# zwyang6/ExCEL

Measured on AMD Instinct MI355X. Metric: images/sec (CAM+PAR refine, 448x448), higher is better.
Workload: dtype bf16x3 (fp32 as bf16 hi+lo, fp32 accumulate)

## Files before the change

### excel_amd/csrc/abi.hip

```cpp
#include "../../include/excel_hip.h"
#include "common.h"
#include "excel_internal.h"

#include <stdarg.h>
#include <map>
#include <vector>

static thread_local char g_err[512] = "";

void excel_set_error(const char* fmt, ...) {
    va_list ap;
    va_start(ap, fmt);
    vsnprintf(g_err, sizeof(g_err), fmt, ap);
    va_end(ap);
}

extern "C" const char* excel_last_error(void) { return g_err; }
extern "C" int excel_abi_version(void) { return 5; }
#ifndef EXCEL_BUILD_ID
#define EXCEL_BUILD_ID "unstamped"
#endif
extern "C" const char* excel_build_id(void) { return EXCEL_BUILD_ID; }

bool g_excel_prof_on = false;
// ... 532 lines not shown

extern "C" size_t excel_cam_workspace_bytes(int B, int N, int T) {
    return align_up((size_t)B * N * ((T + 3) / 4 * 4) * sizeof(float), 256);
}

extern "C" int excel_clip_feature_surgery(const float* image_features, const float* text, int B, int N, int C, int T, int F,
                                          float temperature, float* out_full, float* out_slice, void* workspace, void* stream) {
    EXCEL_CHECK_ARG(image_features && text && workspace && (out_full || out_slice), "clip_feature_surgery: null argument");
    EXCEL_CHECK_ARG((C % 4) == 0, "clip_feature_surgery: C must be a multiple of 4");
    const int ldT = (T + 3) / 4 * 4;
    float* S = (float*)workspace;
    GemmArgs ga = gemm_args(image_features, text, S, nullptr, nullptr, B * N, T, C, C, C, ldT, 0, GEMM_ACT_NONE);
    TRY(excel_launch_gemm(ga, true, 1, ST(stream)));
    return excel_launch_cam_epilogue(S, out_full, out_slice, B, N, T, ldT, F, temperature, ST(stream));
}

struct PtcWs { float *sim, *part, *colsq; unsigned short* ts; size_t total; };
static PtcWs ptc_ws_layout(int B, int N, int C, int T, char* base) {
    PtcWs w;
    size_t off = 0;
    auto take = [&](size_t bytes) { char* p = base + off; off += align_up(bytes, 256); return p; };
    w.sim = (float*)take(excel_patch_text_cam_ws_floats(B, N, C, T, 0) * sizeof(float));
    w.ts = (unsigned short*)take((size_t)T * C * sizeof(float));
    w.part = (float*)take(excel_patch_text_cam_ws_floats(B, N, C, T, 1) * sizeof(float));
    w.colsq = (float*)take(excel_patch_text_cam_ws_floats(B, N, C, T, 2) * sizeof(float));
    w.total = off;
    return w;
}
extern "C" size_t excel_patch_text_cam_workspace_bytes(int B, int N, int C, int T) { return ptc_ws_layout(B, N, C, T, nullptr).total; }

extern "C" int excel_patch_text_cam(const float* x_raw, const float* text, int B, int N, int C, int T, int F, float temperature, int mode,
                                    float* out_full, float* out_slice, float* image_features, void* workspace, void* stream) {
    EXCEL_CHECK_ARG(x_raw && text && workspace && (out_full || out_slice), "patch_text_cam: null argument");
    EXCEL_CHECK_ARG(mode == 0 || mode == 1 || mode == 2, "patch_text_cam: mode must be 0 (exact fp32), 1 (bf16x3) or 2 (f16x3)");
    EXCEL_CHECK_ARG(B > 0 && N > 0 && C > 0 && T > 0, "patch_text_cam: bad shape");
    const int ldT = (T + 3) / 4 * 4;
    const PtcWs w = ptc_ws_layout(B, N, C, T, (char*)workspace);
    if (mode == 2)
        return excel_f16::excel_launch_patch_text_cam(x_raw, text, w.ts, w.sim, w.part, w.colsq, out_full, out_slice, image_features, B, N, C, T, F,
                                                      ldT, temperature, 1, ST(stream));
    return excel_launch_patch_text_cam(x_raw, text, mode == 1 ? w.ts : nullptr, w.sim, w.part, w.colsq, out_full, out_slice, image_features, B, N, C,
                                       T, F, ldT, temperature, mode, ST(stream));
}

extern "C" int excel_attn_layer_mean(const float* attn, int Lw, int B, int N, int first_layer, int n_layers, float* w_aff, void* stream) {
    EXCEL_CHECK_ARG(attn && w_aff && first_layer >= 0 && n_layers >= 1 && first_layer + n_layers <= Lw, "attn_layer_mean: bad layer range");
    const long long n = (long long)B * (N - 1) * (N - 1);
    hipLaunchKernelGGL(attn_layer_mean_kernel, dim3((unsigned)cdivl(n, 256)), dim3(256), 0, ST(stream), attn, B, N, first_layer, n_layers, w_aff);
    EXCEL_CHECK_LAUNCH("attn_layer_mean");
    return EXCEL_OK;
}

extern "C" size_t excel_trans_mat_workspace_bytes(int B, int P) {
    return 2 * align_up((size_t)B * P * P * sizeof(float), 256) + align_up((size_t)B * P * sizeof(float), 256);
}

extern "C" int excel_compute_trans_mat(const float* w_aff, int B, int P, float* trans_out, void* workspace, void* stream) {
    EXCEL_CHECK_ARG(w_aff && trans_out && workspace, "compute_trans_mat: null argument");
    EXCEL_CHECK_ARG((P % 4) == 0, "compute_trans_mat: P must be a multiple of 4 (P=%d)", P);
    char* base = (char*)workspace;
    const size_t mat = align_up((size_t)B * P * P * sizeof(float), 256);
    float* T = (float*)base;
    float* Tsym = (float*)(base + mat);
    float* cs = (float*)(base + 2 * mat);
    TRY(excel_launch_trans_mat_sym(w_aff, T, Tsym, cs, B, P, ST(stream)));
    GemmArgs ga = gemm_args(Tsym, Tsym, trans_out, nullptr, nullptr, P, P, P, P, P, P, 0, GEMM_ACT_NONE);
    ga.sA = ga.sB = ga.sC = (long long)P * P;
    return excel_launch_gemm(ga, true, B, ST(stream));
}

extern "C" int excel_cls_compact(const float* onehot, int B, int F, int Smax, int32_t* cls_idx, int32_t* ncls, int32_t* nchan,
                                 void* stream) {
    EXCEL_CHECK_ARG(onehot && cls_idx && ncls && Smax >= 1, "cls_compact: bad argument");
    return excel_launch_cls_compact(onehot, B, F, Smax, cls_idx, ncls, nchan, ST(stream));
}

extern "C" int excel_scoremap_box_mask(const float* attr, const int32_t* cls_idx, const int32_t* ncls, int B, int g, int F, int Smax,
                                       double caa_thre, float* v_out, uint8_t* mask_out, void* stream) {
    EXCEL_CHECK_ARG(attr && cls_idx && ncls && v_out, "scoremap_box_mask: null argument");
    return excel_launch_bbox_mask(attr, cls_idx, ncls, B, g, F, Smax, caa_thre, v_out, mask_out, ST(stream));
}

extern "C" size_t excel_refine_workspace_bytes(int B, int P, int Smax) {
    return 2 * align_up((size_t)B * P * P * sizeof(float), 256) + align_up((size_t)B * P * sizeof(float), 256) +
           2 * align_up((size_t)B * Smax * P * sizeof(float), 256);
}

extern "C" int excel_refine_cams_with_aff(const float* attr, const float* w_aff, const int32_t* cls_idx, const int32_t* ncls, int B,
                                          int g, int F, int Smax, double caa_thre, float* refined, void* workspace, void* stream) {
    EXCEL_CHECK_ARG(attr && w_aff && cls_idx && ncls && refined && workspace, "refine_cams_with_aff: null argument");
    const int P = g * g;
    char* base = (char*)workspace;
    const size_t mat = align_up((size_t)B * P * P * sizeof(float), 256);
    const size_t vec = align_up((size_t)B * Smax * P * sizeof(float), 256);
    float* T = (float*)base;
    float* Tsym = (float*)(base + mat);
    float* cs = (float*)(base + 2 * mat);
    float* v = (float*)(base + 2 * mat + align_up((size_t)B * P * sizeof(float), 256));
    float* u = (float*)((char*)v + vec);
    hipStream_t st = ST(stream);
    TRY(excel_launch_trans_mat_sym(w_aff, T, Tsym, cs, B, P, st));
    TRY(excel_launch_bbox_mask(attr, cls_idx, ncls, B, g, F, Smax, caa_thre, v, nullptr, st));
    TRY(excel_launch_matvec(Tsym, v, ncls, u, B, P, Smax, st));
    TRY(excel_launch_matvec(Tsym, u, ncls, refined, B, P, Smax, st));
    return EXCEL_OK;
}

extern "C" int excel_cam_upsample_bkg(const float* refined, const int32_t* ncls, int B, int g, int Smax, int H, int W, float* cams,
                                      void* workspace, int flags, void* stream) {
    EXCEL_CHECK_ARG(refined && ncls && cams && workspace, "cam_upsample_bkg: null argument");
    return excel_launch_cam_upsample_bkg(refined, ncls, (float*)workspace, cams, B, g, Smax, H, W, (flags & EXCEL_CAMS_ZERO_UNUSED) ? 1 : 0, ST(stream));
}

extern "C" int excel_ragged_plan(const int32_t* hw, int B, excel_ragged_info* info, int32_t* table) {
    EXCEL_CHECK_ARG(hw && info && B >= 1, "ragged_plan: bad argument");
    long long pix = 0, lab = 0, tiles = 0, max_plane = 0;
    for (int b = 0; b < B; ++b) {
        const long long H = hw[2 * b], W = hw[2 * b + 1];
        EXCEL_CHECK_ARG(H >= 1 && W >= 1, "ragged_plan: image %d has size %lld x %lld", b, H, W);
        const long long Wp = (W + 3) / 4 * 4, plane = H * Wp, nt = ((W + 63) / 64) * ((H + 15) / 16);
        if (table) {
            int32_t* rec = table + EXCEL_RAG_REC * b;
            rec[0] = (int32_t)H; rec[1] = (int32_t)W; rec[2] = (int32_t)pix; rec[3] = (int32_t)tiles; rec[4] = (int32_t)lab; rec[5] = rec[6] = rec[7] = 0;
            for (long long t = 0; t < nt; ++t) table[EXCEL_RAG_REC * (B + 1) + tiles + t] = b;
        }
        pix += plane; lab += H * W; tiles += nt;
        if (plane > max_plane) max_plane = plane;
        EXCEL_CHECK_ARG(pix < (1LL << 31) && 3 * lab < (1LL << 31) && tiles < (1LL << 31), "ragged_plan: batch too large for 32-bit offsets");
    }
    if (table) {
        int32_t* rec = table + EXCEL_RAG_REC * B;
        rec[0] = rec[1] = 0; rec[2] = (int32_t)pix; rec[3] = (int32_t)tiles; rec[4] = (int32_t)lab; rec[5] = rec[6] = rec[7] = 0;
    }
    info->B = B; info->total_tiles = (int32_t)tiles; info->total_pix = pix; info->total_label_pix = lab; info->max_plane_pix = max_plane;
    info->table_ints = EXCEL_RAG_REC * (long long)(B + 1) + tiles;
    return EXCEL_OK;
}

static TileGeo ragged_geo(const int32_t* table, int B) {
    TileGeo g;
    g.tab = table; g.B = B; g.H = g.W = 0;
    return g;
}
static TileGeo uniform_geo(int B, int H, int W) {
    TileGeo g;
    g.tab = nullptr; g.B = B; g.H = H; g.W = W;
    return g;
}

extern "C" int excel_normalize_resize_u8_ragged(const uint8_t* hwc, const int32_t* table, int B, int S, const double* mean3, const double* std3,
                                                float* out, void* stream) {
    EXCEL_CHECK_ARG(hwc && table && out && mean3 && std3 && B > 0 && S > 0, "normalize_resize_u8_ragged: bad argument");
    return excel_launch_normalize_resize_u8_ragged(hwc, out, ragged_geo(table, B), S, mean3, std3, ST(stream));
}

extern "C" int excel_normalize_resize_u8_ragged_mirror(const uint8_t* hwc, const int32_t* table, int B, int S, const double* mean3,
                                                       const double* std3, float* out, void* stream) {
    EXCEL_CHECK_ARG(hwc && table && out && mean3 && std3 && B > 0 && S > 0, "normalize_resize_u8_ragged_mirror: bad argument");
    return excel_launch_normalize_resize_u8_ragged_mirror(hwc, out, ragged_geo(table, B), S, mean3, std3, ST(stream));
}

extern "C" int excel_cam_upsample_bkg_ragged(const float* refined, const int32_t* ncls, const int32_t* table, const excel_ragged_info* info, int g,
                                             int Smax, float* cams, void* workspace, int flags, void* stream) {
    EXCEL_CHECK_ARG(refined && ncls && table && info && cams && workspace, "cam_upsample_bkg_ragged: null argument");
    EXCEL_CHECK_ARG((((uintptr_t)cams) & 15) == 0, "cam_upsample_bkg_ragged: cams must be 16-byte aligned");
    return excel_launch_cam_upsample_bkg_ragged(refined, ncls, (float*)workspace, cams, g, Smax, ragged_geo(table, info->B), info->total_tiles,
                                                (flags & EXCEL_CAMS_ZERO_UNUSED) ? 1 : 0, ST(stream));
}

int excel_aug_plan(const int32_t* hw, const excel_aug_params* prm, int B, int S, excel_train_aug_info* info, int32_t* table);
int excel_launch_train_augment(const unsigned char* hwc, const unsigned char* labels, const int* table, const excel_train_aug_info& info,
                               const double* mean, const double* stdv, float* img, unsigned char* label, int* img_box, void* workspace,
                               hipStream_t st);
int excel_launch_train_augment_image(const unsigned char* hwc, const int* table, const excel_train_aug_info& info, const double* mean,
                                     const double* stdv, float* img, int* img_box, void* workspace, hipStream_t st);
extern "C" int excel_train_aug_plan(const int32_t* hw, const excel_aug_params* params, int B, int S, excel_train_aug_info* info, int32_t* table) {
    return excel_aug_plan(hw, params, B, S, info, table);
}

extern "C" size_t excel_train_augment_workspace_bytes(const excel_train_aug_info* info) {
    return info ? (size_t)info->workspace_bytes : 0;
}

extern "C" int excel_train_augment(const uint8_t* hwc, const uint8_t* labels, const int32_t* table, const excel_train_aug_info* info,
                                   const double* mean3, const double* std3, float* img, uint8_t* label, int32_t* img_box, void* workspace,
                                   void* stream) {
    EXCEL_CHECK_ARG(hwc && labels && table && info && mean3 && std3 && img && label && img_box && workspace, "train_augment: null argument");
    EXCEL_CHECK_ARG(info->B >= 1 && info->S >= 1 && info->max_h >= 1 && info->max_w2 >= 1 && info->workspace_bytes > 0,
// ... 144 lines not shown
```

### excel_amd/csrc/aff.hip

```cpp
#include "common.h"
#include "excel_internal.h"

__global__ __launch_bounds__(256) void colsum_kernel(const float* __restrict__ T, float* __restrict__ cs, int P) {
    __shared__ float part[4][64];
    const int b = blockIdx.y, cl = threadIdx.x & 63, g = threadIdx.x >> 6;
    const int c = blockIdx.x * 64 + cl;
    const float* Tb = T + (long long)b * P * P;
    float a8[8] = {0.f, 0.f, 0.f, 0.f, 0.f, 0.f, 0.f, 0.f};
    if (c < P) {
        int i = g;
        for (; i + 28 < P; i += 32) {
#pragma unroll
            for (int u = 0; u < 8; ++u) a8[u] += Tb[(long long)(i + 4 * u) * P + c];
        }
        for (int u = 0; i < P; i += 4, ++u) a8[u] += Tb[(long long)i * P + c];
    }
    const float s = ((a8[0] + a8[1]) + (a8[2] + a8[3])) + ((a8[4] + a8[5]) + (a8[6] + a8[7]));
    part[g][cl] = s;
    __syncthreads();
    if (g == 0 && c < P) cs[(long long)b * P + c] = (part[0][cl] + part[1][cl]) + (part[2][cl] + part[3][cl]);
}

#define SK_MAXP 2048
__global__ __launch_bounds__(256) void sinkhorn_row_kernel(const float* __restrict__ in, const float* __restrict__ cs,
// ... 67 lines not shown
    const int cls = cls_idx[(long long)b * Smax + s];
    const int P = g * g;
    if (tid == 0) { s_max = 0; s_nroots = 0; }
    __syncthreads();
    int u8v[BB_MAXP / 256];
#pragma unroll
    for (int k = 0; k < BB_MAXP / 256; ++k) {
        const int p = tid + 256 * k;
        u8v[k] = 0;
        if (p < P) {
            const float x = attr[((long long)b * P + p) * F + cls];
            gv[p] = x;
            u8v[k] = (int)(x * 255.f) & 255;
            atomicMax(&s_max, u8v[k]);
        }
    }
    __syncthreads();
    const int thr = (int)(thre * (double)s_max);
#pragma unroll
    for (int k = 0; k < BB_MAXP / 256; ++k) {
        const int p = tid + 256 * k;
        if (p < P) {
            lab[p] = (u8v[k] > thr) ? p : -1;
            bx0[p] = g; bx1[p] = -1; by0[p] = g; by1[p] = -1;
        }
    }
    __syncthreads();
    for (int iter = 0; iter < 2 * BB_MAXP; ++iter) {
        if (tid == 0) s_changed = 0;
        __syncthreads();
#pragma unroll
        for (int k = 0; k < BB_MAXP / 256; ++k) {
            const int p = tid + 256 * k;
            if (p < P && lab[p] >= 0) {
                const int y = p / g, x = p % g;
                int best = lab[p];
                for (int dy = -1; dy <= 1; ++dy)
                    for (int dx = -1; dx <= 1; ++dx) {
                        const int yy = y + dy, xx = x + dx;
                        if (yy >= 0 && yy < g && xx >= 0 && xx < g) {
                            const int l2 = lab[yy * g + xx];
                            if (l2 >= 0 && l2 < best) best = l2;
                        }
                    }
                const int jump = lab[best];
                if (jump >= 0 && jump < best) best = jump;
                if (best < lab[p]) { atomicMin(&lab[p], best); s_changed = 1; }
            }
        }
        __syncthreads();
        if (!s_changed) break;
        __syncthreads();
    }
#pragma unroll
    for (int k = 0; k < BB_MAXP / 256; ++k) {
        const int p = tid + 256 * k;
        if (p < P && lab[p] >= 0) {
            const int root = lab[p], y = p / g, x = p % g;
            atomicMin(&bx0[root], x); atomicMax(&bx1[root], x);
            atomicMin(&by0[root], y); atomicMax(&by1[root], y);
            if (root == p) roots[atomicAdd(&s_nroots, 1)] = p;
        }
    }
    __syncthreads();
    const int nroots = s_nroots;
#pragma unroll
    for (int k = 0; k < BB_MAXP / 256; ++k) {
        const int p = tid + 256 * k;
        if (p < P) {
            const int y = p / g, x = p % g;
            bool in = false;
            for (int i = 0; i < nroots; ++i) {
                const int rt = roots[i];
                const int x1 = min(bx1[rt] + 1, g - 1), y1 = min(by1[rt] + 1, g - 1);
                in = in || (x >= bx0[rt] && x < x1 && y >= by0[rt] && y < y1);
            }
            v_out[((long long)b * Smax + s) * P + p] = in ? gv[p] : 0.f;
            if (mask_out) mask_out[((long long)b * Smax + s) * P + p] = in ? 1 : 0;
        }
    }
}

#define MV_S 8
__global__ __launch_bounds__(256) void matvec_kernel(const float* __restrict__ T, const float* __restrict__ v,
                                                     const int* __restrict__ ncls, float* __restrict__ u, int P, int Smax,
                                                     int s0) {
    extern __shared__ float vs[];
    const int b = blockIdx.y;
    const int ns = min(min(ncls[b], Smax) - s0, MV_S);
    if (ns <= 0) return;
    for (int i = threadIdx.x; i < ns * P; i += 256) vs[i] = v[((long long)b * Smax + s0) * P + i];
    __syncthreads();
    const int lane = threadIdx.x & 63, wave = threadIdx.x >> 6;
    for (int rr = 0; rr < 4; ++rr) {
        const int i = blockIdx.x * 16 + wave * 4 + rr;
        if (i >= P) break;
        const float* row = T + ((long long)b * P + i) * P;
        float acc[MV_S];
#pragma unroll
        for (int s = 0; s < MV_S; ++s) acc[s] = 0.f;
        for (int j = lane; j < P; j += 64) {
            const float t = row[j];
#pragma unroll
            for (int s = 0; s < MV_S; ++s)
                if (s < ns) acc[s] += t * vs[s * P + j];
        }
#pragma unroll
        for (int s = 0; s < MV_S; ++s) {
            if (s < ns) {
                const float r = wave_sum(acc[s]);
                if (lane == 0) u[((long long)b * Smax + s0 + s) * P + i] = r;
            }
        }
    }
}

__global__ __launch_bounds__(256) void cam_minmax_norm_kernel(const float* __restrict__ r, const int* __restrict__ ncls,
                                                              float* __restrict__ rn, int P, int Smax) {
    __shared__ float smn[4], smx[4];
    const int s = blockIdx.x, b = blockIdx.y;
    if (s >= min(ncls[b], Smax)) return;
    const float* src = r + ((long long)b * Smax + s) * P;
    float mn = INFINITY, mx = -INFINITY;
    for (int p = threadIdx.x; p < P; p += 256) { const float v = src[p]; mn = fminf(mn, v); mx = fmaxf(mx, v); }
    mn = wave_min(mn); mx = wave_max(mx);
    if ((threadIdx.x & 63) == 0) { smn[threadIdx.x >> 6] = mn; smx[threadIdx.x >> 6] = mx; }
    __syncthreads();
    mn = fminf(fminf(smn[0], smn[1]), fminf(smn[2], smn[3]));
    mx = fmaxf(fmaxf(smx[0], smx[1]), fmaxf(smx[2], smx[3]));
    const float den = 1e-7f + (mx - mn);
    float* dst = rn + ((long long)b * Smax + s) * P;
    for (int p = threadIdx.x; p < P; p += 256) dst[p] = (src[p] - mn) / den;
}

struct CvTap { int s0, s1; float f; };
__device__ __forceinline__ CvTap cv_linear_tap(int d, int g, int D) {
    const double fd = ((double)d + 0.5) * ((double)g / (double)D) - 0.5;
    CvTap t;
    t.s0 = (int)floor(fd);
    t.f = (float)(fd - t.s0);
    if (t.s0 < 0) { t.f = 0.f; t.s0 = 0; }
    if (t.s0 >= g - 1) { t.f = 0.f; t.s0 = g - 1; }
    t.s1 = min(t.s0 + 1, g - 1);
    return t;
}
__device__ __forceinline__ void cam_upsample_px(const float* __restrict__ rn_b, float* __restrict__ out, long long HW, int g, int ns, int Smax,
                                                const CvTap& tx, const CvTap& ty, int zero_unused) {
    float mx = -INFINITY;
    for (int s = 0; s < ns; ++s) {
        const float* m = rn_b + (long long)s * g * g;
        const float top = fmaf(m[ty.s0 * g + tx.s1], tx.f, __fmul_rn(m[ty.s0 * g + tx.s0], 1.f - tx.f));
        const float bot = fmaf(m[ty.s1 * g + tx.s1], tx.f, __fmul_rn(m[ty.s1 * g + tx.s0], 1.f - tx.f));
        const float v = fmaf(bot, ty.f, __fmul_rn(top, 1.f - ty.f));
        out[(long long)(s + 1) * HW] = v;
        mx = fmaxf(mx, v);
    }
    out[0] = 1.f - mx;
    if (zero_unused)
        for (int s = ns; s < Smax; ++s) out[(long long)(s + 1) * HW] = 0.f;
}

__global__ __launch_bounds__(256) void cam_upsample_bkg_kernel(const float* __restrict__ rn, const int* __restrict__ ncls,
                                                               float* __restrict__ cams, int g, int Smax, int H, int W, int zero_unused) {
    const int b = blockIdx.z;
    const int x = blockIdx.x * 64 + (threadIdx.x & 63);
    const int y = blockIdx.y * 4 + (threadIdx.x >> 6);
    if (x >= W || y >= H) return;
    const int ns = min(ncls[b], Smax);
    const long long HW = (long long)H * W;
    cam_upsample_px(rn + (long long)b * Smax * g * g, cams + (long long)b * (Smax + 1) * HW + (long long)y * W + x, HW, g, ns, Smax,
                    cv_linear_tap(x, g, W), cv_linear_tap(y, g, H), zero_unused);
}

__global__ __launch_bounds__(256) void cam_upsample_bkg_ragged_kernel(const float* __restrict__ rn, const int* __restrict__ ncls,
                                                                      float* __restrict__ cams, int g, int Smax, TileGeo geo, int zero_unused) {
    const Tile t = tile_of<true>(geo);
    const int x = t.x0 + (threadIdx.x & 63);
    if (x >= t.W) return;
    const int ns = min(ncls[t.b], Smax);
    const CvTap tx = cv_linear_tap(x, g, t.W);
    const float* rn_b = rn + (long long)t.b * Smax * g * g;
    float* cb = cams + (long long)(Smax + 1) * t.base + x;
#pragma unroll 1
    for (int r = 0; r < 4; ++r) {
        const int y = t.y0 + (threadIdx.x >> 6) + 4 * r;
        if (y < t.H) cam_upsample_px(rn_b, cb + (long long)y * t.Wp, t.HW, g, ns, Smax, tx, cv_linear_tap(y, g, t.H), zero_unused);
    }
}

int excel_launch_trans_mat_sym(const float* W, float* T, float* Tsym, float* cs, int B, int P, hipStream_t st) {
    ProfScope prof__(PROF_SINKHORN, st);
    EXCEL_CHECK_ARG(P <= SK_MAXP, "compute_trans_mat: P=%d exceeds %d", P, SK_MAXP);
    const float* src = W;
    for (int round = 0; round < 3; ++round) {
        hipLaunchKernelGGL(colsum_kernel, dim3(cdiv(P, 64), B), dim3(256), 0, st, src, cs, P);
        hipLaunchKernelGGL(sinkhorn_row_kernel, dim3(cdiv(P, 4), B), dim3(256), 0, st, src, cs, T, P);
        src = T;
    }
    hipLaunchKernelGGL(symmetrize_kernel, dim3(cdiv(P, 32), cdiv(P, 32), B), dim3(256), 0, st, T, Tsym, P);
    EXCEL_CHECK_LAUNCH("trans_mat_sym");
    return EXCEL_OK;
}

int excel_launch_cls_compact(const float* onehot, int B, int F, int Smax, int* cls_idx, int* ncls, int* nchan, hipStream_t st) {
    ProfScope prof__(PROF_OTHER, st);
    hipLaunchKernelGGL(cls_compact_kernel, dim3(cdiv(B, 64)), dim3(64), 0, st, onehot, B, F, Smax, cls_idx, ncls, nchan);
    EXCEL_CHECK_LAUNCH("cls_compact");
    return EXCEL_OK;
}

int excel_launch_bbox_mask(const float* attr, const int* cls_idx, const int* ncls, int B, int g, int F, int Smax, double thre,
                           float* v_out, unsigned char* mask_out, hipStream_t st) {
    ProfScope prof__(PROF_BBOX, st);
    EXCEL_CHECK_ARG(g * g <= BB_MAXP, "scoremap2bbox: grid %dx%d exceeds %d cells", g, g, BB_MAXP);
    hipLaunchKernelGGL(bbox_mask_kernel, dim3(Smax, B), dim3(256), 0, st, attr, cls_idx, ncls, g, F, Smax, thre, v_out, mask_out);
    EXCEL_CHECK_LAUNCH("bbox_mask");
    return EXCEL_OK;
}

int excel_launch_matvec(const float* T, const float* v, const int* ncls, float* u, int B, int P, int Smax, hipStream_t st) {
    ProfScope prof__(PROF_MATVEC, st);
    for (int s0 = 0; s0 < Smax; s0 += MV_S) {
        hipLaunchKernelGGL(matvec_kernel, dim3(cdiv(P, 16), B), dim3(256), MV_S * P * sizeof(float), st, T, v, ncls, u, P, Smax, s0);
    }
    EXCEL_CHECK_LAUNCH("matvec");
    return EXCEL_OK;
}

int excel_launch_cam_upsample_bkg(const float* r, const int* ncls, float* rn, float* cams, int B, int g, int Smax, int H, int W,
                                  int zero_unused, hipStream_t st) {
    ProfScope prof__(PROF_UPSAMPLE, st);
    hipLaunchKernelGGL(cam_minmax_norm_kernel, dim3(Smax, B), dim3(256), 0, st, r, ncls, rn, g * g, Smax);
    hipLaunchKernelGGL(cam_upsample_bkg_kernel, dim3(cdiv(W, 64), cdiv(H, 4), B), dim3(256), 0, st, rn, ncls, cams, g, Smax, H, W, zero_unused);
    EXCEL_CHECK_LAUNCH("cam_upsample_bkg");
    return EXCEL_OK;
}

int excel_launch_cam_upsample_bkg_ragged(const float* r, const int* ncls, float* rn, float* cams, int g, int Smax, const TileGeo& geo,
                                         int total_tiles, int zero_unused, hipStream_t st) {
    ProfScope prof__(PROF_UPSAMPLE, st);
    hipLaunchKernelGGL(cam_minmax_norm_kernel, dim3(Smax, geo.B), dim3(256), 0, st, r, ncls, rn, g * g, Smax);
    hipLaunchKernelGGL(cam_upsample_bkg_ragged_kernel, dim3(total_tiles), dim3(256), 0, st, rn, ncls, cams, g, Smax, geo, zero_unused);
    EXCEL_CHECK_LAUNCH("cam_upsample_bkg_ragged");
    return EXCEL_OK;
}
```

### excel_amd/csrc/excel_internal.h

```cpp
#pragma once
#include <hip/hip_runtime.h>

enum { GEMM_ACT_NONE = 0, GEMM_ACT_QUICKGELU = 1, GEMM_ACT_RELU = 2 };
enum { GEMM_OUT_PLAIN = 0, GEMM_OUT_QKV_HEADMAJOR = 1, GEMM_OUT_SPLIT_BF16 = 2 };

struct GemmArgs {
    const float* A;
    const float* B;
    float* C;
    const float* bias;
    const float* res;
    int M, N, K;
    int Kld;
    int lda, ldb, ldc, ldr;
    long long sA, sB, sC, sR, sBias;
    int zdiv;
    long long sA2, sB2, sC2;
    int act;
    int out_mode;
    int tokN, heads, hd;
    float alpha;
};


// ... 2 lines not shown
    const unsigned short* B;
    float* C;
    unsigned short* Cs;
    const float* bias;
    const float* res;
    int M, N, K;
    int lda, ldb, ldc, ldr;
    int act, out_mode;
    int tokN, heads, hd;
    unsigned short* qkv_split;
    int dbg;
    int batch;
    long long sA, sB, sC, sCs;
    int mix_tall, mix_short;
    int mix_first;
    int w_lo_zero;
    const unsigned short* Bh;
    int ldbh;
};

struct GemmShape {
    int M, N, K, lda, ldb, ldc, ldr, hd, out_mode, has_residual, batch;
    int f16;
    int w_lo_zero;
    int half_ok;
};
enum { GEMM_8WAVE = 0, GEMM_8WAVE_MIXED = 1, GEMM_W4 = 2, GEMM_W4_MIX = 3 };
struct GemmPlan {
    int kernel;
    int tile;
    int nt_m;
    int x2;
    int tall, shrt, second;
    int grid_x, grid_y, block;
};
constexpr int GEMM_W4_BN = 256;
GemmPlan gemm_plan(const GemmShape& s, int n_cu);
enum { ATTN_STRIP = 0, ATTN_TWOPASS_SPLIT = 1, ATTN_TWOPASS_F32 = 2 };
constexpr int ATTN_STRIP_MAX_TILES = 40;
struct AttnPlan {
    int path;
    int ntiles;
    int ntw, nw, nw_full;
    int rp_ntypes;
    int rp_grid[3];
    int grid[3], block;
    int split_c;
};
AttnPlan attn_plan(int B, int H, int N, int gemm_mode, int surgery, int want_w);
enum { CAM_NARROW = 0, CAM_WIDE = 1 };
constexpr int PTC_MAXCT = 4;
constexpr int PTC_WIDE_T = 512;
constexpr int PTC_NW = 4;
constexpr int PTC_HB = 64;
constexpr int PTC_TLDS_ROWS = 48;
constexpr int PTC_TLDS_C = 512;
struct CamPlan {
    int kernel;
    int split;
    int ct;
    int tlds;
    int G;
    int prep_grid[3];
    int sim_grid[2], block;
    int finish_grid[2];
    int finish_pitch;
};
CamPlan cam_plan(int B, int N, int C, int T, int gemm_mode);
inline bool gemm_half_ok(bool aligned, int N, int K, int ldbh) {
    return aligned && ldbh >= K && (ldbh & 7) == 0 && (long long)N * ldbh * 2 < 0x7fffffffLL;
}

int excel_launch_gemm(const GemmArgs& p, bool b_kmajor, int batch, hipStream_t stream);
int excel_launch_attn_rowpass_f32(const float* qkvh, float* out, float* stats, int B, int H, int N, int hd, float scale,
                                  const AttnPlan& plan, hipStream_t st, int flash_nq);
int excel_launch_attn_accum_f32(const float* qkvh, const float* stats, float* a_sum, float* w_aff, float* attn_out, int B, int H,
                                int N, int NP, int hd, float scale, int surgery, float w_scale, float aff_scale, int aff_init,
                                const AttnPlan& plan, hipStream_t st, const float* ex_attn);

int excel_launch_trans_mat_sym(const float* W, float* T, float* Tsym, float* cs, int B, int P, hipStream_t st);
int excel_launch_cls_compact(const float* onehot, int B, int F, int Smax, int* cls_idx, int* ncls, int* nchan, hipStream_t st);
int excel_launch_bbox_mask(const float* attr, const int* cls_idx, const int* ncls, int B, int g, int F, int Smax, double thre,
                           float* v_out, unsigned char* mask_out, hipStream_t st);
int excel_launch_matvec(const float* T, const float* v, const int* ncls, float* u, int B, int P, int Smax, hipStream_t st);
int excel_launch_cam_upsample_bkg(const float* r, const int* ncls, float* rn, float* cams, int B, int g, int Smax, int H, int W,
                                  int zero_unused, hipStream_t st);
struct TileGeo;
int excel_launch_par_affinity(const float* img, float* aff, const TileGeo& geo, int total_tiles, const int* dil, int ndil, float w1, float w2,
                              hipStream_t st, int compact = 0);
int excel_par_guide_supported(const void* guide, const void* stats, const void* in, const void* out, int Cmax, long long max_plane, int Wp,
                              const int* dil, int ndil);
int excel_launch_par_iterate_guide(const float* guide, const float* stats, const float* in, float* out, const int* nchan, int Cmax,
                                   const TileGeo& geo, int total_tiles, const int* dil, int ndil, float w1, float w2, hipStream_t st);
int excel_launch_par_iterate(const float* aff, const float* in, float* out, const int* nchan, int B, int Cmax, int H, int W,
                             const int* dil, int ndil, hipStream_t st);
int excel_launch_bilinear_ac_ragged(const float* in, float* out, int h, int w, const TileGeo& geo, int total_tiles, hipStream_t st);
int excel_launch_argmax_label_ragged(const float* cams, const int* nchan, const int* cls_idx, int Smax, int Cmax, const TileGeo& geo,
                                     int total_tiles, unsigned char* lab8, hipStream_t st);
int excel_launch_cam_upsample_bkg_ragged(const float* r, const int* ncls, float* rn, float* cams, int g, int Smax, const TileGeo& geo,
                                         int total_tiles, int zero_unused, hipStream_t st);
int excel_launch_normalize_resize_u8_ragged(const unsigned char* hwc, float* out, const TileGeo& geo, int S, const double* mean, const double* stdv,
                                            hipStream_t st);
int excel_launch_normalize_resize_u8_ragged_mirror(const unsigned char* hwc, float* out, const TileGeo& geo, int S, const double* mean,
                                                   const double* stdv, hipStream_t st);
int excel_launch_bilinear_ac(const float* in, float* out, int planes, int h, int w, int H, int W, hipStream_t st);
int excel_launch_argmax_label(const float* cams, const int* nchan, const int* cls_idx, int B, int Smax, int Cmax, long long HW,
                              unsigned char* lab8, long long* lab64, hipStream_t st);
int excel_launch_confusion(const unsigned char* gt, const unsigned char* pred, long long n, int nc, unsigned long long* hist,
                           hipStream_t st);
int excel_launch_attr_aggregate(const float* text, const float* bank, int F, int T, int C, int K, int drop, float* out,
                                hipStream_t st);
int excel_launch_bilinear_resize(const float* in, float* out, long long planes, int h, int w, int H, int W, int align_corners,
                                 hipStream_t st);
int excel_launch_flip_max_normalize(const float* attr, float* out, int B, int g, int F, hipStream_t st);
int excel_launch_lam_scale_accumulate(const float* maps, float* acc, int B, int g, int F, int H, int W, int init, hipStream_t st);
int excel_launch_plane_minmax_normalize(float* lam, long long planes, long long HW, hipStream_t st);
int excel_launch_seg_scale_accumulate(const float* segs, float* acc, int B, int nc, int h, int w, int H, int W, int flip_mean, int init,
                                      float scale, hipStream_t st);
int excel_launch_denormalize(const float* img, unsigned char* out8, float* outf, int B, long long HW, const float* mean, const float* stdv,
                             hipStream_t st);
int excel_launch_normalize_u8(const unsigned char* hwc, float* out, int B, long long HW, const double* mean, const double* stdv, hipStream_t st);
int excel_launch_lam_to_label(const float* cam, const float* cls, const int* box, int B, int F, int H, int W, float bkg, float high, float low,
                              int ignore_mid, int ignore, float* valid, unsigned char* lab, hipStream_t st);
size_t excel_train_losses_ws_bytes(int B, int nc, int H, int W);
int excel_launch_train_losses(const float* seg, const float* attn_pred, const unsigned char* pseudo, const unsigned char* aff_labels, int B, int nc,
                              int g_h, int g_w, int H, int W, int radius, int ignore, float w_seg, float w_diver, float* losses, float* d_seg,
                              float* d_attn_pred, void* ws, hipStream_t st);
size_t excel_feature_affinity_ws_bytes(int B, int C, int P);
int excel_launch_feature_affinity(const float* feats, int B, int C, int P, float beta, float gamma, int mode, float* out, void* ws,
                                  hipStream_t st);
size_t excel_feature_affinity_grouped_ws_bytes(int B, int C, int P, int group);
int excel_launch_feature_affinity_grouped(const float* feats, int B, int C, int P, int group, int member_stride, float beta, float gamma,
                                          int mode, float* out, void* ws, hipStream_t st);
size_t excel_attn_select_ws_bytes(int B, int n_layers);
int excel_launch_attn_select_mean(const float* attn, int Lw, int B, int N, int first_layer, int n_layers, const float* seg_attn,
                                  float* out, void* ws, hipStream_t st);

namespace excel_bf16 {
#include "excel_split_api.inc"
}
namespace excel_f16 {
#include "excel_split_api.inc"
}
#ifdef EXCEL_SPLIT_F16
#define EXCEL_SPLIT_NS excel_f16
#else
#define EXCEL_SPLIT_NS excel_bf16
#endif
using namespace excel_bf16;

struct BilinearTap { int y0, y1, x0, x1; float ly, lx; };
__device__ __forceinline__ BilinearTap bilinear_tap(int x, int y, int h, int w, int H, int W, int align_corners) {
    float fy, fx;
    if (align_corners) {
        fy = ((H > 1) ? (float)(h - 1) / (float)(H - 1) : 0.f) * (float)y;
        fx = ((W > 1) ? (float)(w - 1) / (float)(W - 1) : 0.f) * (float)x;
    } else {
        fy = fmaxf(__fsub_rn(__fmul_rn((float)h / (float)H, (float)y + 0.5f), 0.5f), 0.f);
        fx = fmaxf(__fsub_rn(__fmul_rn((float)w / (float)W, (float)x + 0.5f), 0.5f), 0.f);
    }
    BilinearTap t;
    t.y0 = min((int)fy, h - 1); t.x0 = min((int)fx, w - 1);
    t.y1 = min(t.y0 + 1, h - 1); t.x1 = min(t.x0 + 1, w - 1);
    t.ly = fy - (float)t.y0; t.lx = fx - (float)t.x0;
    return t;
}
__device__ __forceinline__ float bilinear_blend(const BilinearTap& t, float p00, float p01, float p10, float p11) {
// ... 5 lines not shown
```

Before: 1493.

## Fuse Sinkhorn normalization and symmetrization into on-the-fly random-walk passes

Replaces the materialized transition matrix T and symmetric Tsym (two B×P×P buffers built by trans_mat_sym) with streaming passes over the raw affinity W. The passes compute row and column normalizers on the fly and apply the symmetric average as (row-half + column-half)/2, using per-block partial sums and a finish kernel. This removes the P×P intermediate writes and reads and the separate matvec kernel. In exchange it rereads W several times, adds more launches and partial-sum buffers, and reorders the floating-point arithmetic.

```diff
diff --git a/excel_amd/csrc/abi.hip b/excel_amd/csrc/abi.hip
--- a/excel_amd/csrc/abi.hip
+++ b/excel_amd/csrc/abi.hip
@@ -638,28 +638,14 @@
 }
 
 extern "C" size_t excel_refine_workspace_bytes(int B, int P, int Smax) {
-    return 2 * align_up((size_t)B * P * P * sizeof(float), 256) + align_up((size_t)B * P * sizeof(float), 256) +
-           2 * align_up((size_t)B * Smax * P * sizeof(float), 256);
+    return excel_refine_walk_workspace_bytes(B, P, Smax);
 }
 
 extern "C" int excel_refine_cams_with_aff(const float* attr, const float* w_aff, const int32_t* cls_idx, const int32_t* ncls, int B,
                                           int g, int F, int Smax, double caa_thre, float* refined, void* workspace, void* stream) {
     EXCEL_CHECK_ARG(attr && w_aff && cls_idx && ncls && refined && workspace, "refine_cams_with_aff: null argument");
-    const int P = g * g;
-    char* base = (char*)workspace;
-    const size_t mat = align_up((size_t)B * P * P * sizeof(float), 256);
-    const size_t vec = align_up((size_t)B * Smax * P * sizeof(float), 256);
-    float* T = (float*)base;
-    float* Tsym = (float*)(base + mat);
-    float* cs = (float*)(base + 2 * mat);
-    float* v = (float*)(base + 2 * mat + align_up((size_t)B * P * sizeof(float), 256));
-    float* u = (float*)((char*)v + vec);
-    hipStream_t st = ST(stream);
-    TRY(excel_launch_trans_mat_sym(w_aff, T, Tsym, cs, B, P, st));
-    TRY(excel_launch_bbox_mask(attr, cls_idx, ncls, B, g, F, Smax, caa_thre, v, nullptr, st));
-    TRY(excel_launch_matvec(Tsym, v, ncls, u, B, P, Smax, st));
-    TRY(excel_launch_matvec(Tsym, u, ncls, refined, B, P, Smax, st));
-    return EXCEL_OK;
+    EXCEL_CHECK_ARG(B >= 1 && g >= 1 && Smax >= 1, "refine_cams_with_aff: bad shape");
+    return excel_launch_refine_walk(attr, w_aff, cls_idx, ncls, B, g, F, Smax, caa_thre, refined, workspace, ST(stream));
 }
 
 extern "C" int excel_cam_upsample_bkg(const float* refined, const int32_t* ncls, int B, int g, int Smax, int H, int W, float* cams,
diff --git a/excel_amd/csrc/aff.hip b/excel_amd/csrc/aff.hip
--- a/excel_amd/csrc/aff.hip
+++ b/excel_amd/csrc/aff.hip
@@ -173,37 +173,180 @@
 }
 
 #define MV_S 8
-__global__ __launch_bounds__(256) void matvec_kernel(const float* __restrict__ T, const float* __restrict__ v,
-                                                     const int* __restrict__ ncls, float* __restrict__ u, int P, int Smax,
-                                                     int s0) {
-    extern __shared__ float vs[];
-    const int b = blockIdx.y;
-    const int ns = min(min(ncls[b], Smax) - s0, MV_S);
-    if (ns <= 0) return;
-    for (int i = threadIdx.x; i < ns * P; i += 256) vs[i] = v[((long long)b * Smax + s0) * P + i];
-    __syncthreads();
-    const int lane = threadIdx.x & 63, wave = threadIdx.x >> 6;
-    for (int rr = 0; rr < 4; ++rr) {
-        const int i = blockIdx.x * 16 + wave * 4 + rr;
-        if (i >= P) break;
-        const float* row = T + ((long long)b * P + i) * P;
-        float acc[MV_S];
-#pragma unroll
-        for (int s = 0; s < MV_S; ++s) acc[s] = 0.f;
-        for (int j = lane; j < P; j += 64) {
-            const float t = row[j];
-#pragma unroll
-            for (int s = 0; s < MV_S; ++s)
-                if (s < ns) acc[s] += t * vs[s * P + j];
-        }
-#pragma unroll
-        for (int s = 0; s < MV_S; ++s) {
-            if (s < ns) {
-                const float r = wave_sum(acc[s]);
-                if (lane == 0) u[((long long)b * Smax + s0 + s) * P + i] = r;
-            }
-        }
-    }
+#define RW_WAVE_ROWS 8
+__device__ __forceinline__ float walk_colsum(const float* __restrict__ p, int n, long long stride) {
+    float a = 0.f;
+    int k = 0;
+    for (; k + 4 <= n; k += 4) {
+        const float t0 = p[k * stride], t1 = p[(k + 1) * stride], t2 = p[(k + 2) * stride], t3 = p[(k + 3) * stride];
+        a = (((a + t0) + t1) + t2) + t3;
+    }
+    for (; k < n; ++k) a += p[k * stride];
+    return a;
+}
+
+template <int RB, int NK>
+__device__ __forceinline__ void walk_load_rows(float (&t)[RB][NK], const float* __restrict__ W, int b, int P, int i0, int lane) {
+#pragma unroll
+    for (int q = 0; q < RB; ++q) {
+        const int i = i0 + q;
+        const float* row = W + ((long long)b * P + min(i, P - 1)) * P;
+#pragma unroll
+        for (int k = 0; k < NK; ++k) {
+            const int j = lane + 64 * k;
+            t[q][k] = (64 * k < P && j < P && i < P) ? row[j] : 0.f;
+        }
+    }
+}
+
+template <bool RINV, bool HASX, int NK, int THREADS>
+__global__ __launch_bounds__(THREADS, (HASX || NK > 13) ? 2 : 4) void walk_pass_kernel(
+    const float* __restrict__ W, const float* __restrict__ cin, int nin, float* r, const float* __restrict__ x, const int* __restrict__ ncls,
+    float* __restrict__ rowhalf, float* __restrict__ part, int P, int Smax, int s0) {
+    extern __shared__ float lds[];
+    constexpr int NS = HASX ? 4 : 1, SLOTS = HASX ? MV_S : 1;
+    constexpr int RB = HASX ? 2 : 4;
+    constexpr bool PREFETCH = HASX;
+    constexpr int ROWS = THREADS / 64 * RW_WAVE_ROWS;
+    const int b = blockIdx.y, blk = blockIdx.x, nblk = gridDim.x, tid = threadIdx.x;
+    int ns = 1;
+    if (HASX) {
+        ns = min(min(ncls[b], Smax) - s0, MV_S);
+        if (ns <= 0) return;
+    }
+    float* cs = lds;
+    float* cxs = lds + P;
+    float* red = lds + (1 + ns) * P;
+    float* rrow = red + NS * P;
+    float* xrow = rrow + ROWS;
+    const float* xb = HASX ? x + ((long long)b * Smax + s0) * P : nullptr;
+    for (int j = tid; j < P; j += THREADS) {
+        const float c = 1.f / walk_colsum(cin + (long long)b * nin * P + j, nin, P);
+        cs[j] = c;
+        if (HASX)
+            for (int s = 0; s < ns; ++s) cxs[s * P + j] = c * xb[s * P + j];
+    }
+    if (HASX) {
+        for (int e = tid; e < (1 + ns) * ROWS; e += THREADS) {
+            const int s = e / ROWS - 1, i = blk * ROWS + e % ROWS;
+            if (s >= 0) rrow[e] = (i < P) ? xb[s * P + i] : 0.f;
+            else if (!RINV) rrow[e] = (i < P) ? r[(long long)b * P + i] : 0.f;
+        }
+    }
+    __syncthreads();
+    const int lane = tid & 63, wave = tid >> 6;
+    const int l0 = wave * RW_WAVE_ROWS, i0 = blk * ROWS + l0;
+    for (int sb = 0; sb < ns; sb += NS) {
+        float cacc[NS][NK];
+#pragma unroll
+        for (int s = 0; s < NS; ++s)
+#pragma unroll
+            for (int k = 0; k < NK; ++k) cacc[s][k] = 0.f;
+        float t[RB][NK], tn[RB][NK];
+        if (PREFETCH) walk_load_rows<RB, NK>(t, W, b, P, i0, lane);
+        for (int rr = 0; rr < RW_WAVE_ROWS; rr += RB) {
+            if (PREFETCH) {
+                if (rr + RB < RW_WAVE_ROWS) walk_load_rows<RB, NK>(tn, W, b, P, i0 + rr + RB, lane);
+            } else {
+                walk_load_rows<RB, NK>(t, W, b, P, i0 + rr, lane);
+            }
+            float d[RB], dx[RB][NS];
+#pragma unroll
+            for (int q = 0; q < RB; ++q) {
+                d[q] = 0.f;
+#pragma unroll
+                for (int s = 0; s < NS; ++s) dx[q][s] = 0.f;
+            }
+            if (RINV) {
+#pragma unroll
+                for (int k = 0; k < NK; ++k)
+                    if (64 * k < P) {
+                        const float c = cs[min(lane + 64 * k, P - 1)];
+#pragma unroll
+                        for (int q = 0; q < RB; ++q) d[q] = fmaf(t[q][k], c, d[q]);
+                    }
+            }
+            if (HASX) {
+#pragma unroll
+                for (int s = 0; s < NS; ++s)
+                    if (sb + s < ns) {
+#pragma unroll
+                        for (int k = 0; k < NK; ++k)
+                            if (64 * k < P) {
+                                const float cx = cxs[(sb + s) * P + min(lane + 64 * k, P - 1)];
+#pragma unroll
+                                for (int q = 0; q < RB; ++q) dx[q][s] = fmaf(t[q][k], cx, dx[q][s]);
+                            }
+                    }
+            }
+#pragma unroll
+            for (int q = 0; q < RB; ++q) {
+                if (RINV) d[q] = wave_sum(d[q]);
+                if (HASX) {
+#pragma unroll
+                    for (int s = 0; s < NS; ++s) dx[q][s] = wave_sum(dx[q][s]);
+                }
+            }
+#pragma unroll
+            for (int q = 0; q < RB; ++q) {
+                const int li = l0 + rr + q, i = i0 + rr + q;
+                const bool live = i < P;
+                float ri = 0.f;
+                if (RINV) {
+                    if (live) ri = 1.f / d[q];
+                    if (live && lane == 0 && sb == 0) r[(long long)b * P + i] = ri;
+                } else {
+                    ri = rrow[li];
+                }
+#pragma unroll
+                for (int s = 0; s < NS; ++s) {
+                    if (sb + s < ns && live) {
+                        float w = ri;
+                        if (HASX) {
+                            if (lane == 0) rowhalf[((long long)b * Smax + s0 + sb + s) * P + i] = ri * dx[q][s];
+                            w = ri * xrow[(sb + s) * ROWS + li];
+                        }
+#pragma unroll
+                        for (int k = 0; k < NK; ++k) cacc[s][k] = fmaf(t[q][k], w, cacc[s][k]);
+                    }
+                }
+            }
+            if (PREFETCH) {
+#pragma unroll
+                for (int q = 0; q < RB; ++q)
+#pragma unroll
+                    for (int k = 0; k < NK; ++k) t[q][k] = tn[q][k];
+            }
+        }
+        const int nv = min(ns - sb, NS);
+        for (int w = 0; w < THREADS / 64; ++w) {
+            if (wave == w) {
+#pragma unroll
+                for (int s = 0; s < NS; ++s)
+                    if (s < nv) {
+#pragma unroll
+                        for (int k = 0; k < NK; ++k) {
+                            const int j = lane + 64 * k;
+                            if (j < P) red[s * P + j] = (w == 0) ? cacc[s][k] : red[s * P + j] + cacc[s][k];
+                        }
+                    }
+            }
+            __syncthreads();
+        }
+        float* dst = part + (((long long)b * nblk + blk) * SLOTS + sb) * P;
+        for (int e = tid; e < nv * P; e += THREADS) dst[e] = red[e];
+        __syncthreads();
+    }
+}
+
+__global__ __launch_bounds__(256) void walk_apply_fin_kernel(const float* __restrict__ part, const float* __restrict__ cin, int nin,
+                                                             const int* __restrict__ ncls, float* __restrict__ y, int P, int nblk, int Smax,
+                                                             int s0) {
+    const int b = blockIdx.z, s = blockIdx.y, j = blockIdx.x * 256 + threadIdx.x;
+    if (j >= P || s >= min(min(ncls[b], Smax) - s0, MV_S)) return;
+    const float a = walk_colsum(part + ((long long)b * nblk * MV_S + s) * P + j, nblk, (long long)MV_S * P);
+    float* dst = y + ((long long)b * Smax + s0 + s) * P + j;
+    *dst = (*dst + (1.f / walk_colsum(cin + (long long)b * nin * P + j, nin, P)) * a) / 2.f;
 }
 
 __global__ __launch_bounds__(256) void cam_minmax_norm_kernel(const float* __restrict__ r, const int* __restrict__ ncls,
@@ -309,12 +452,62 @@
     return EXCEL_OK;
 }
 
-int excel_launch_matvec(const float* T, const float* v, const int* ncls, float* u, int B, int P, int Smax, hipStream_t st) {
+template <bool RINV, bool HASX>
+static void walk_pass(int B, int nvec, hipStream_t st, const float* W, const float* cin, int nin, float* r, const float* x,
+                      const int* ncls, float* rowhalf, float* part, int P, int Smax, int s0) {
+    constexpr int THREADS = HASX ? 256 : 512, ROWS = THREADS / 64 * RW_WAVE_ROWS;
+    const dim3 grid(cdiv(P, ROWS), B);
+    const size_t lds = ((size_t)(1 + nvec + (HASX ? 4 : 1)) * P + (1 + nvec) * ROWS) * sizeof(float);
+    if (P <= 13 * 64)
+        hipLaunchKernelGGL((walk_pass_kernel<RINV, HASX, 13, THREADS>), grid, dim3(THREADS), lds, st, W, cin, nin, r, x, ncls, rowhalf, part, P, Smax, s0);
+    else
+        hipLaunchKernelGGL((walk_pass_kernel<RINV, HASX, 16, THREADS>), grid, dim3(THREADS), lds, st, W, cin, nin, r, x, ncls, rowhalf, part, P, Smax, s0);
+}
+
+static size_t walk_ws_region(size_t floats) { return (floats * sizeof(float) + 255) / 256 * 256; }
+
+size_t excel_refine_walk_workspace_bytes(int B, int P, int Smax) {
+    const size_t nsink = cdiv(P, 8 * RW_WAVE_ROWS), napp = cdiv(P, 4 * RW_WAVE_ROWS);
+    return 2 * walk_ws_region((size_t)B * P) + 2 * walk_ws_region(B * nsink * P) + 2 * walk_ws_region((size_t)B * Smax * P) +
+           walk_ws_region(B * napp * MV_S * P);
+}
+
+int excel_launch_refine_walk(const float* attr, const float* W, const int* cls_idx, const int* ncls, int B, int g, int F, int Smax,
+                             double thre, float* refined, void* workspace, hipStream_t st) {
+    const int P = g * g, nsink = cdiv(P, 8 * RW_WAVE_ROWS), napp = cdiv(P, 4 * RW_WAVE_ROWS);
+    EXCEL_CHECK_ARG(P <= BB_MAXP, "refine_cams_with_aff: grid %dx%d exceeds %d cells", g, g, BB_MAXP);
+    char* base = (char*)workspace;
+    const size_t vecP = walk_ws_region((size_t)B * P), sink = walk_ws_region((size_t)B * nsink * P), vecS = walk_ws_region((size_t)B * Smax * P);
+    float* cden = (float*)base;
+    float* sinkA = (float*)(base + vecP);
+    float* sinkB = (float*)(base + vecP + sink);
+    float* r = (float*)(base + vecP + 2 * sink);
+    float* v = (float*)(base + 2 * vecP + 2 * sink);
+    float* u = (float*)((char*)v + vecS);
+    float* part = (float*)((char*)u + vecS);
+    {
+        ProfScope prof__(PROF_SINKHORN, st);
+        hipLaunchKernelGGL(colsum_kernel, dim3(cdiv(P, 64), B), dim3(256), 0, st, W, cden, P);
+        walk_pass<true, false>(B, 1, st, W, cden, 1, r, nullptr, ncls, nullptr, sinkA, P, Smax, 0);
+        walk_pass<true, false>(B, 1, st, W, sinkA, nsink, r, nullptr, ncls, nullptr, sinkB, P, Smax, 0);
+        EXCEL_CHECK_LAUNCH("refine_walk sinkhorn");
+    }
+    if (const int rc = excel_launch_bbox_mask(attr, cls_idx, ncls, B, g, F, Smax, thre, v, nullptr, st)) return rc;
     ProfScope prof__(PROF_MATVEC, st);
     for (int s0 = 0; s0 < Smax; s0 += MV_S) {
-        hipLaunchKernelGGL(matvec_kernel, dim3(cdiv(P, 16), B), dim3(256), MV_S * P * sizeof(float), st, T, v, ncls, u, P, Smax, s0);
-    }
-    EXCEL_CHECK_LAUNCH("matvec");
+        const int nvec = min(Smax - s0, MV_S);
+        if (s0 == 0)
+            walk_pass<true, true>(B, nvec, st, W, sinkB, nsink, r, v, ncls, u, part, P, Smax, s0);
+        else
+            walk_pass<false, true>(B, nvec, st, W, sinkB, nsink, r, v, ncls, u, part, P, Smax, s0);
+        hipLaunchKernelGGL(walk_apply_fin_kernel, dim3(cdiv(P, 256), nvec, B), dim3(256), 0, st, part, sinkB, nsink, ncls, u, P, napp, Smax, s0);
+    }
+    for (int s0 = 0; s0 < Smax; s0 += MV_S) {
+        const int nvec = min(Smax - s0, MV_S);
+        walk_pass<false, true>(B, nvec, st, W, sinkB, nsink, r, u, ncls, refined, part, P, Smax, s0);
+        hipLaunchKernelGGL(walk_apply_fin_kernel, dim3(cdiv(P, 256), nvec, B), dim3(256), 0, st, part, sinkB, nsink, ncls, refined, P, napp, Smax, s0);
+    }
+    EXCEL_CHECK_LAUNCH("refine_walk");
     return EXCEL_OK;
 }
 
diff --git a/excel_amd/csrc/excel_internal.h b/excel_amd/csrc/excel_internal.h
--- a/excel_amd/csrc/excel_internal.h
+++ b/excel_amd/csrc/excel_internal.h
@@ -108,7 +108,9 @@
 int excel_launch_cls_compact(const float* onehot, int B, int F, int Smax, int* cls_idx, int* ncls, int* nchan, hipStream_t st);
 int excel_launch_bbox_mask(const float* attr, const int* cls_idx, const int* ncls, int B, int g, int F, int Smax, double thre,
                            float* v_out, unsigned char* mask_out, hipStream_t st);
-int excel_launch_matvec(const float* T, const float* v, const int* ncls, float* u, int B, int P, int Smax, hipStream_t st);
+size_t excel_refine_walk_workspace_bytes(int B, int P, int Smax);
+int excel_launch_refine_walk(const float* attr, const float* W, const int* cls_idx, const int* ncls, int B, int g, int F, int Smax,
+                             double thre, float* refined, void* workspace, hipStream_t st);
 int excel_launch_cam_upsample_bkg(const float* r, const int* ncls, float* rn, float* cams, int B, int g, int Smax, int H, int W,
                                   int zero_unused, hipStream_t st);
 struct TileGeo;
diff --git a/tools_dev/refine_stage_table.py b/tools_dev/refine_stage_table.py
--- /dev/null
+++ b/tools_dev/refine_stage_table.py
@@ -0,0 +1,13 @@
+import sqlite3, sys
+db, steps, label = sqlite3.connect(sys.argv[1]), int(sys.argv[2]), sys.argv[3]
+KEYS = ("colsum_kernel", "sinkhorn_row_kernel", "symmetrize_kernel", "matvec_kernel", "bbox_mask_kernel", "walk_pass_kernel", "walk_colsum_fin_kernel", "walk_apply_fin_kernel")
+rows = db.execute("select name, count(*), sum(duration), avg(duration), min(duration), max(duration) from kernels group by name order by sum(duration) desc").fetchall()
+rows = [r for r in rows if any(k in r[0] for k in KEYS)]
+print(f"# {label}: rocprofv3 --kernel-trace of `bench.py --gpus 1 --steps {steps - 2} --warmup 2` ({steps} steps, B = 32, 448^2); random-walk launches only")
+print(f"{'kernel':<72} {'calls':>6} {'calls/step':>10} {'total_ms':>10} {'avg_us':>10} {'min_us':>10} {'max_us':>10} {'us/step':>9}")
+tot = 0
+for name, n, t, avg, mn, mx in rows:
+    short = name if len(name) <= 72 else name[:69] + "..."
+    print(f"{short:<72} {n:>6} {n / steps:>10.2f} {t / 1e6:>10.3f} {avg / 1e3:>10.2f} {mn / 1e3:>10.2f} {mx / 1e3:>10.2f} {t / 1e3 / steps:>9.1f}")
+    tot += t
+print(f"{'random-walk stage, sum of launches':<72} {sum(r[1] for r in rows):>6} {sum(r[1] for r in rows) / steps:>10.2f} {tot / 1e6:>10.3f} {'':>10} {'':>10} {'':>10} {tot / 1e3 / steps:>9.1f}")
diff --git a/tools_dev/refine_walk_bench.py b/tools_dev/refine_walk_bench.py
--- /dev/null
+++ b/tools_dev/refine_walk_bench.py
@@ -0,0 +1,38 @@
+import os, sys, subprocess
+here = os.path.dirname(os.path.dirname(os.path.abspath(__file__)))
+if sys.argv[1] == "--one":
+    sys.path.insert(0, here)
+    import numpy as np, torch
+    from excel_amd import _lib
+    _lib.LIB_PATH = os.path.abspath(sys.argv[3])
+    from excel_amd import ops
+    rs = np.random.RandomState(0)
+    B, g, F, smax = 32, 28, 20, 6
+    P = g * g
+    sys.path.insert(0, os.path.join(here, "tests"))
+    from test_gpu_ops import _smooth_maps
+    attr = torch.from_numpy(_smooth_maps(rs, B, g, F)).cuda()
+    w = torch.rand(B, P, P, device="cuda") ** 6 + 1e-4
+    onehot = np.zeros((B, F), np.float32)
+    ks = rs.choice([int(k) for k in os.environ.get("MB_KS", "1,1,1,2,2,2,3,3,4,5").split(",")], B)
+    for b in range(B):
+        onehot[b, rs.choice(F, ks[b], replace=False)] = 1
+    idx, ncls = ops.cls_compact(torch.from_numpy(onehot).cuda(), smax)
+    for _ in range(5):
+        out = ops.refine_cams_with_aff_batched(attr, w, idx, ncls, g, 0.79)
+    torch.cuda.synchronize()
+    res = []
+    for rep in range(5):
+        e0, e1 = torch.cuda.Event(enable_timing=True), torch.cuda.Event(enable_timing=True)
+        e0.record()
+        for _ in range(40):
+            out = ops.refine_cams_with_aff_batched(attr, w, idx, ncls, g, 0.79)
+        e1.record(); torch.cuda.synchronize()
+        res.append(e0.elapsed_time(e1) / 40 * 1e3)
+    print(f"{sys.argv[2]:<12} us/call {' '.join('%.1f' % r for r in res)}  mean classes {ks.mean():.2f}  checksum {float(out.double().sum()):.9e}", flush=True)
+else:
+    a = sys.argv[1:]
+    for label, path in zip(a[0::2], a[1::2]):
+        rc = subprocess.run(["timeout", "-k", "10", "120", sys.executable, os.path.abspath(__file__), "--one", label, path]).returncode
+        if rc != 0:
+            print("stopped:", label, "rc", rc); sys.exit(rc)
```

New measurement: 1499 (median of 6 runs). No clear change (+0.4%).
